# espiriki/Garbage_Classification_RCA

Hardware: AMD Instinct MI355X
Metric: train samples/sec (image+text pairs), MM-RCA ViT-B16+DistilBERT (higher is better)
Workload: dtype bf16

## Files before the change

garbage_classification_rca_amd/csrc/gemm256.hip:

```cpp
#include "common.h"
#include "lds_asm.h"
#include <type_traits>
#include <mutex>

typedef __attribute__((ext_vector_type(4))) float f32x4;
typedef __attribute__((address_space(3))) void lds_void;
typedef const __attribute__((address_space(1))) void gbl_void;

#define HT_BYTES (128 * 64 * 2)
#define STAGE_BYTES (4 * HT_BYTES)
#define LDS256_BYTES (128 * (256 * 4 + 16))
#define SLOT_A0 0
#define SLOT_A1 1
#define SLOT_B0 2
#define SLOT_B1 3

__device__ __forceinline__ int krow_f2(int row) { return (row & 3) | (((row >> 3) & 1) << 2); }

__device__ __forceinline__ void stage_half(const bf16_t* src0, const bf16_t* src1, char* lds_piece0) {
  __builtin_amdgcn_global_load_lds((gbl_void*)src0, (lds_void*)(lds_piece0), 16, 0, 0);
  __builtin_amdgcn_global_load_lds((gbl_void*)src1, (lds_void*)(lds_piece0 + 1024), 16, 0, 0);
}

template <bool F4>
__device__ __forceinline__ void stage_half_t(const bf16_t* src0, const bf16_t* src1, char* lds_piece0) {
  __builtin_amdgcn_global_load_lds((gbl_void*)src0, (lds_void*)(lds_piece0), 16, 0, 0);
  __builtin_amdgcn_global_load_lds((gbl_void*)src1, (lds_void*)(lds_piece0 + (F4 ? 8192 : 1024)), 16, 0, 0);
}

template <bool KROW, bool STRIPE = false>
__device__ __forceinline__ const bf16_t* piece_src(const bf16_t* __restrict__ base, int64_t ld, int64_t row0, int64_t rows_total,
                                                   int i, int lane, int h = 0) {
  if (!KROW) {
    const int r = 8 * i + (lane >> 3);
    const int c = (lane & 7) ^ ((r >> 1) & 7);
    int64_t gr = row0 + (STRIPE ? 64 * (r >> 5) + 32 * h + (r & 31) : r);
// ... 818 lines not shown
                       lda, ldb, ldc, tiles_m, tiles_n, ksteps_base, ksteps_rem, (float*)workspace, (float*)nullptr, splits,    \
                       (const bf16_t*)A_lo, (const bf16_t*)B_lo, nseg);                                                         \
  } while (0)
  if (x3) {
    if (!ak && !bk) LSLAB(false, false, true);
    else if (!ak && bk) LSLAB(false, true, true);
    else if (ak && !bk) LSLAB(true, false, true);
    else LSLAB(true, true, true);
  } else {
    if (!ak && !bk) LSLAB(false, false, false);
    else if (!ak && bk) LSLAB(false, true, false);
    else if (ak && !bk) LSLAB(true, false, false);
    else LSLAB(true, true, false);
  }
#undef LSLAB
  MMRCA_CHECK_LAUNCH("gemm_splitk(mfma256)");
  hipLaunchKernelGGL(splitk_reduce256_k, dim3(tiles * 64), dim3(256), 0, st, (const float*)workspace, C, ldc, tiles, tiles_n, splits, M, N);
  MMRCA_CHECK_LAUNCH("gemm_splitk(reduce)");
  return 0;
}

extern "C" int mmrca_gemm_splitk(const void* A, const void* B, float* C, void* workspace, int64_t workspace_bytes, int64_t M,
                                 int64_t N, int64_t K, int64_t lda, int64_t ldb, int64_t ldc, int a_layout, int b_layout,
                                 void* stream) {
  return gemm_splitk_impl(A, nullptr, B, nullptr, C, workspace, workspace_bytes, M, N, K, lda, ldb, ldc, a_layout, b_layout, stream);
}

extern "C" int mmrca_gemm_splitk_x3(const void* A_hi, const void* A_lo, const void* B_hi, const void* B_lo, float* C, void* workspace,
                                    int64_t workspace_bytes, int64_t M, int64_t N, int64_t K, int64_t lda, int64_t ldb, int64_t ldc,
                                    int a_layout, int b_layout, void* stream) {
  MMRCA_REQUIRE(A_lo || !B_lo, "gemm_x3(splitk): a B lo plane without an A lo plane is not a supported pass set");
  return gemm_splitk_impl(A_hi, A_lo, B_hi, B_lo, C, workspace, workspace_bytes, M, N, K, lda, ldb, ldc, a_layout, b_layout, stream);
}
```

garbage_classification_rca_amd/engine.py:

```python
from __future__ import annotations

import math
import os
import re
from typing import Dict, List, Optional, Tuple

import torch

from . import lib as L
from . import spec as S
from .conv_engine import ConvEncoder, CONV_MODELS

ALIGN = 64
CONCURRENT_ENCODERS = os.environ.get("MMRCA_CONCURRENT_ENCODERS", "1") == "1"
CLS_TAIL = os.environ.get("MMRCA_CLS_TAIL", "1") == "1"
X3_WGRAD_PASSES = int(os.environ.get("MMRCA_X3_WGRAD_PASSES", "3"))
X3_DGRAD_PASSES = int(os.environ.get("MMRCA_X3_DGRAD_PASSES", "3"))
ROWPAD = 256


def _round_up(x: int, m: int) -> int:
    return (x + m - 1) // m * m


class Arena:
    def __init__(self, entries: List[Tuple[str, Tuple[int, ...]]], device, with_lp: bool, with_lo: bool = False):
        self.offsets: Dict[str, Tuple[int, Tuple[int, ...], int]] = {}
        off = 0
        for k, shp in entries:
            n = 1
            for s in shp:
                n *= s
            off = _round_up(off, ALIGN)
            self.offsets[k] = (off, tuple(shp), n)
            off += n
        self.total = _round_up(off, ALIGN)
        self.p = torch.zeros(self.total, dtype=torch.float32, device=device)
        self.g = torch.zeros(self.total, dtype=torch.float32, device=device)
        self.lp = torch.zeros(self.total, dtype=torch.bfloat16, device=device) if with_lp else None
        self.lp_lo = torch.zeros(self.total, dtype=torch.bfloat16, device=device) if with_lo else None
        self.lp_valid = False
        self._views: Dict[Tuple[str, str], torch.Tensor] = {}

    def view(self, key, which="p"):
        v = self._views.get((key, which))
        if v is None:
            off, shp, n = self.offsets[key]
            v = self._views[(key, which)] = getattr(self, which)[off:off + n].view(shp)
# ... 285 lines not shown
                elif is_norm:
                    v.fill_(1.0 if leaf == "weight" else 0.0)
                elif is_head:
                    if v.dim() == 2:
                        bound = 1.0 / math.sqrt(v.shape[1])
                        v.copy_((torch.rand(v.shape, generator=g) * 2 - 1) * bound)
                        self._last_fan_in = v.shape[1]
                    else:
                        bound = 1.0 / math.sqrt(self._last_fan_in)
                        v.copy_((torch.rand(v.shape, generator=g) * 2 - 1) * bound)
                elif leaf == "bias" or leaf.endswith("_bias"):
                    v.zero_()
                else:
                    v.copy_(torch.randn(v.shape, generator=g) * 0.02)
        self.arena.lp_valid = False

    def load_arrays(self, sd: Dict[str, "torch.Tensor"], strict=True):
        with torch.no_grad():
            for k in self.param_keys:
                if k in sd:
                    self.arena.view(k).copy_(torch.as_tensor(sd[k]).to(self.device, torch.float32).view(self.arena.offsets[k][1]))
                elif strict:
                    raise KeyError(k)
        self.arena.lp_valid = False

    def _splitk_ws(self):
        key = ("splitk_ws", torch.cuda.current_stream().cuda_stream)
        t = self._bufs.get(key)
        if t is None:
            t = torch.empty(L.SPLITK_WS_BYTES, dtype=torch.uint8, device=self.device)
            self._bufs[key] = t
        return t

    def vec(self, name, n, dtype=torch.float32, layer=0):
        key = (name, layer, "vec", n, dtype)
        t = self._bufs.get(key)
        if t is None:
            t = self._bufs[key] = torch.zeros(1, n, dtype=dtype, device=self.device)
        return t

    def buf(self, name, rows, cols, dtype=None, layer=0):
        dtype = dtype or self.dtype
        key = (name, layer, rows, cols, dtype)
        t = self._bufs.get(key)
        if t is None:
            t = torch.zeros(_round_up(max(rows, 1), ROWPAD), cols, dtype=dtype, device=self.device)
            self._bufs[key] = t
        return t

    def release_buffers(self):
        self.buffer_generation += 1
        self._bufs.clear()
        self._plane_valid.clear()
        self._plane_fresh.clear()
        self._saved = None
        if self.conv is not None:
            self.conv.release()

    def _lin_fwd(self, x, wkey, bkey, out, M, N, K, act=L.ACT_NONE, preact=None, addend=None, wnumel=None):
        if self.x3:
            b = self.arena.view(bkey) if wnumel is None else self.arena.p[self.arena.offsets[bkey][0]:self.arena.offsets[bkey][0] + N]
            po = isinstance(out, Planes)
            L.gemm_x3(self._split(x, M, K), self.Wx3(wkey, wnumel), out.hi if po else out, C_lo=(out.lo if po else None), bias=b, addend=addend,
                      preact=preact, M=M, N=N, K=K, lda=K, ldb=K, ldc=N, a_layout=L.ROWK, b_layout=L.ROWK, act=act, impl=self.gemm_impl)
            return
        w = self.W(wkey) if wnumel is None else self.Wflat(wkey, wnumel)
        b = self.W(bkey) if wnumel is None else self.Wflat(bkey, N)
        L.gemm(x, w, out, bias=b, addend=addend, preact=preact, M=M, N=N, K=K, lda=K, ldb=K, ldc=N,
               a_layout=L.ROWK, b_layout=L.ROWK, act=act, dtype=self.dt, impl=self.gemm_impl)

    def _lin_bwd(self, dy, x, wkey, bkey, dx, M, N, K, addend=None, wnumel=None, gelu_h=None, bias_done=False, gelu_db=None):
        Mk = _round_up(M, 64)
        gw = self.G(wkey) if wnumel is None else self.Gflat(wkey, wnumel)
        gb = self.G(bkey) if wnumel is None else self.Gflat(bkey, N)
        if self.x3 and not self.x3f:
            return self._lin_bwd_x3(dy, x, wkey, dx, M, N, K, Mk, gw, gb, addend, wnumel, gelu_h, bias_done, gelu_db)
        if self.x3f:
            x = self._hi(x, M, K)
        bdt = self.bdt
        if self.gemm_impl == L.IMPL_AUTO and L.gemm_splitk_ok(N, K, Mk, bdt):
            L.gemm_splitk(dy, x, gw, self._splitk_ws(), M=N, N=K, K=Mk, lda=N, ldb=K, ldc=K)
        else:
            L.gemm(dy, x, gw, M=N, N=K, K=Mk, lda=N, ldb=K, ldc=K, a_layout=L.KROW, b_layout=L.KROW, accum=True, dtype=bdt,
                   impl=self.gemm_impl)
        if not bias_done:
            L.colsum_accum(dy, gb, M, N, N, bdt)
        if dx is not None:
            w = self.Wb(wkey, wnumel)
            fuse = gelu_h is not None
            L.gemm(dy, w, dx, addend=addend, preact=(gelu_h if fuse else None), M=M, N=K, K=N, lda=N, ldb=K, ldc=K,
                   a_layout=L.ROWK, b_layout=L.KROW, act=(L.ACT_MUL if fuse else L.ACT_NONE), dtype=bdt,
                   impl=self.gemm_impl, colsum=(gelu_db if fuse else None))

    def _lin_bwd_x3(self, dy, x, wkey, dx, M, N, K, Mk, gw, gb, addend, wnumel, gelu_h, bias_done, gelu_db):
        dyp = self._split(dy, M, N)
        xp = self._split(x, M, K, reuse=True)
        wg_a, wg_b = (dyp, xp) if X3_WGRAD_PASSES >= 3 else ((dyp, (xp[0], None)) if X3_WGRAD_PASSES == 2 else ((dyp[0], None), (xp[0], None)))
        if self.gemm_impl == L.IMPL_AUTO and L.gemm_splitk_ok(N, K, Mk, L.BF16):
            L.gemm_splitk_x3(wg_a, wg_b, gw, self._splitk_ws(), M=N, N=K, K=Mk, lda=N, ldb=K, ldc=K)
        else:
            L.gemm_x3(wg_a, wg_b, gw, M=N, N=K, K=Mk, lda=N, ldb=K, ldc=K, a_layout=L.KROW, b_layout=L.KROW, accum=True)
        if not bias_done:
            if isinstance(dy, Planes):
                raise L.MmrcaError("bf16x3: the bias gradient of a two-plane dY must come from its producer (bias_done)")
            L.colsum_accum(dy, gb, M, N, N, self.dt)
        if dx is not None:
            fuse = gelu_h is not None
            po = isinstance(dx, Planes)
            wp = self.Wx3(wkey, wnumel)
            dg_a, dg_b = (dyp, wp) if X3_DGRAD_PASSES >= 3 else ((dyp, (wp[0], None)) if X3_DGRAD_PASSES == 2 else ((dyp[0], None), (wp[0], None)))
            L.gemm_x3(dg_a, dg_b, dx.hi if po else dx, C_lo=(dx.lo if po else None), addend=addend,
                      preact=(gelu_h if fuse else None), colsum=(gelu_db if fuse else None),
                      M=M, N=K, K=N, lda=N, ldb=K, ldc=K, a_layout=L.ROWK, b_layout=L.KROW, act=(L.ACT_MUL if fuse else L.ACT_NONE),
                      impl=self.gemm_impl)

    def _ln_fwd(self, x, res, pfx, sum_out, y, mean, rstd, rows, D, eps, ld_x=None, ld_y=None, in_drop=(0.0, 0), out_drop=(0.0, 0),
                to_gemm=False):
# ... 109 lines not shown
                h, g = cb("h", Fd, self._hdt), (self.planes_buf("t_g_c", B, Fd, i if save else 0) if self._g_planes else cb("g", Fd))
                self._lin_fwd(x1, P + K["f1"] + ".weight", P + K["f1"] + ".bias", g, B, Fd, D, act=self._gelu_act, preact=h)
                f = cb("f", D)
                self._lin_fwd(g, P + K["f2"] + ".weight", P + K["f2"] + ".bias", f, B, D, Fd)
                s2, xn = cb("s2", D), cb("xout", D)
                m2, r2 = stat("m2c", i), stat("r2c", i)
                self._ln_fwd(f, x1, P + K["ln2"], s2, xn, m2, r2, B, D, s.ln_eps, in_drop=(dp, sd(i, 3)))
                layers.append(dict(x=x, qkv=qkv, ctx=ctx, lse=lse, s1=s1, x1=x1, m1=m1, r1=r1, h=h, g=g, s2=s2, m2=m2, r2=r2,
                                   ctx_c=ctx_c, tail=True))
                cls = xn[:B].clone()
                return cls, dict(B=B, T=T, M=M, cu=cu, first=first, ids32=ids32, pos=pos, mask32=mask32, emb=emb, mean0=mean0, rstd0=rstd0, layers=layers,
                                 drop_p=dp, drop_seed=drop_seed, taps=tap_rows)
            self._mha_fwd(qkv, mask32, ctx, lse, B, H, T, dh, drop_p=dp, drop_seed=sd(i, 1), cu=cu)
            att = fb("tmpD", D)
            self._lin_fwd(ctx, P + K["o"] + ".weight", P + K["o"] + ".bias", att, M, D, D)
            s1, x1 = fb("s1", D, i), fb("x1", D, i)
            m1, r1 = stat("m1", i), stat("r1", i)
            self._ln_fwd(att, x, P + K["ln1"], s1, x1, m1, r1, M, D, s.ln_eps, in_drop=(post_attn_drop, sd(i, 2)), to_gemm=True)
            h, g = fb("h", Fd, i, self._hdt), (self.planes_buf("t_g", cap, Fd, i if save else 0) if self._g_planes else fb("g", Fd, i))
            self._lin_fwd(x1, P + K["f1"] + ".weight", P + K["f1"] + ".bias", g, M, Fd, D, act=self._gelu_act, preact=h)
            f = fb("tmpD", D)
            self._lin_fwd(g, P + K["f2"] + ".weight", P + K["f2"] + ".bias", f, M, D, Fd)
            s2, xn = fb("s2", D, i), fb("x", D, i + 1)
            m2, r2 = stat("m2", i), stat("r2", i)
            self._ln_fwd(f, x1, P + K["ln2"], s2, xn, m2, r2, M, D, s.ln_eps, in_drop=(dp, sd(i, 3)), to_gemm=(i + 1 < s.layers))
            layers.append(dict(x=x, qkv=qkv, ctx=ctx, lse=lse, s1=s1, x1=x1, m1=m1, r1=r1, h=h, g=g, s2=s2, m2=m2, r2=r2))
            x = xn
            if taps and (i + 1) in taps:
                tap_rows[i + 1] = x.index_select(0, first)
        cls = x.index_select(0, first)
        return cls, dict(B=B, T=T, M=M, cu=cu, first=first, ids32=ids32, pos=pos, mask32=mask32, emb=emb, mean0=mean0, rstd0=rstd0, layers=layers,
                         drop_p=dp, drop_seed=drop_seed, taps=tap_rows)

    def _text_upper_backward(self, dy, sv, i, K, rows, cap, sfx):
        s, P = self.ts, "text_model."
        D, Fd = s.dim, s.ffn
        a = sv["layers"][i]
        gb = lambda name, cols: self.buf("tg_" + name + sfx, cap, cols, self.gdtype)
        dp, sd = sv["drop_p"], (lambda layer, site: self._site_seed(sv["drop_seed"], layer, site))
        post_attn_drop = dp if s.name != "distilbert" else 0.0
        ds2 = gb("ds2", D)
        df = gb("dbr_ffn", D) if dp > 0 else None
        gb_f2, gb_o = self.G(P + K["f2"] + ".bias"), self.G(P + K["o"] + ".bias")
        self._ln_bwd(dy, a["s2"], P + K["ln2"], a["m2"], a["r2"], None, ds2, rows, D, branch_drop=(dp, sd(i, 3)), dbranch=df,
                     dcol=(None if df is not None else gb_f2), dcol_branch=(gb_f2 if df is not None else None))
        dg = self.planes_buf("tg_dF" + sfx, cap, Fd) if (self._g_planes and not self.x3f) else gb("dF", Fd)
        self._lin_bwd(df if df is not None else ds2, a["g"], P + K["f2"] + ".weight", P + K["f2"] + ".bias", dg, rows, D, Fd,
                      gelu_h=a["h"], bias_done=True, gelu_db=self.G(P + K["f1"] + ".bias"))
        dx1 = gb("dxB", D)
        self._lin_bwd(dg, a["x1"], P + K["f1"] + ".weight", P + K["f1"] + ".bias", dx1, rows, Fd, D, addend=ds2, bias_done=True)
        ds1 = gb("ds1", D)
        datt = gb("dbr_att", D) if post_attn_drop > 0 else None
        self._ln_bwd(dx1, a["s1"], P + K["ln1"], a["m1"], a["r1"], None, ds1, rows, D, branch_drop=(post_attn_drop, sd(i, 2)), dbranch=datt,
                     dcol=(None if datt is not None else gb_o), dcol_branch=(gb_o if datt is not None else None))
        dctx = gb("dctx", D)
        self._lin_bwd(datt if datt is not None else ds1, a["ctx_c" if sfx else "ctx"], P + K["o"] + ".weight", P + K["o"] + ".bias", dctx,
                      rows, D, D, bias_done=True)
        return ds1, dctx

    def _text_backward(self, dcls, sv, dtaps=None):
        s, P = self.ts, "text_model."
        B, T = sv["B"], sv["T"]
        M, D, H = sv["M"], s.dim, s.heads
        dh, cu, first = D // H, sv["cu"], sv["first"]
        gb = lambda name, cols: self.buf("tg_" + name, B * T, cols, self.gdtype)
        dx = gb("dxA", D)
        tail = bool(sv["layers"][-1].get("tail"))
        if not tail:
            dx[:M].zero_()
            dx.index_copy_(0, first, dcls.to(dx.dtype))
        for i in reversed(range(s.layers)):
            if tail and i == s.layers - 1:
                self._text_backward_tail(dcls, sv, dx)
                continue
            K, a = S.text_layer_keys(s, i), sv["layers"][i]
            if dtaps and (i + 1) in dtaps:
                dx.index_add_(0, first, dtaps[i + 1].to(dx.dtype))
            ds1, dctx = self._text_upper_backward(dx, sv, i, K, M, B * T, "")
            dqkv = gb("dqkv", 3 * D)
            qkv_b, ctx_b = self._attn_bwd_operands(a, M, D, "tg", B * T, B)
            L.mha_bwd(qkv_b, sv["mask32"], ctx_b, dctx, a["lse"], dqkv, B, H, T, dh, dh ** -0.5, self.bdt, self.attn_impl,
                      drop_p=sv["drop_p"], drop_seed=self._site_seed(sv["drop_seed"], i, 1), cu=cu)
            self._lin_bwd(dqkv, a["x"], P + K["q"] + ".weight", P + K["q"] + ".bias", dx, M, 3 * D, D, addend=ds1, wnumel=3 * D * D)
            self._ready(f"text_layer_{i}")
        ds0 = gb("ds2", D)
        self._ln_bwd(dx, sv["emb"], P + "embeddings.LayerNorm", sv["mean0"], sv["rstd0"], None, ds0, M, D,
                     dy_drop=(sv["drop_p"], self._site_seed(sv["drop_seed"], 0, 0)))
        dtype_row = self.Gflat(P + "embeddings.token_type_embeddings.weight", D) if s.type_vocab else None
        L.embed_bwd(ds0, sv["ids32"], sv["pos"], self.G(P + "embeddings.word_embeddings.weight"),
                    self.G(P + "embeddings.position_embeddings.weight"), dtype_row, M, D, self.bdt,
                    pad_id=s.pad_id, pos_pad_id=(s.pad_id if s.pos_offset else -1))
        self._ready("text_emb", flush=True)

    def _text_backward_tail(self, dcls, sv, dx):
        s, P = self.ts, "text_model."
        B, T = sv["B"], sv["T"]
        M, D, H = sv["M"], s.dim, s.heads
        dh, i, cu, first = D // H, s.layers - 1, sv["cu"], sv["first"]
        K, a = S.text_layer_keys(s, i), sv["layers"][i]
        gb = lambda name, cols: self.buf("tg_" + name, B * T, cols, self.gdtype)
        dxc = self.buf("tg_dx_c", B, D, self.gdtype)
        dxc[:B].copy_(dcls)
        ds1, dctx_c = self._text_upper_backward(dxc, sv, i, K, B, B, "_c")
        ds1_full = gb("ds1", D)
        ds1_full[:M].zero_()
        ds1_full.index_copy_(0, first, ds1[:B])
        dqkv = gb("dqkv", 3 * D)
        qkv_b, ctx_b = self._attn_bwd_operands(a, M, D, "tg", B * T, B)
        L.mha_cls_bwd(qkv_b, sv["mask32"], ctx_b, dctx_c, a["lse"], dqkv, B, H, T, dh, dh ** -0.5, self.bdt,
                      drop_p=sv["drop_p"], drop_seed=self._site_seed(sv["drop_seed"], i, 1), cu=cu)
        self._lin_bwd(dqkv, a["x"], P + K["q"] + ".weight", P + K["q"] + ".bias", dx, M, 3 * D, D, addend=ds1_full, wnumel=3 * D * D)
        self._ready(f"text_layer_{i}")

    def _vision_forward(self, images, save):
        s, P = self.vs, "image_model."
        B = images.shape[0]
# ... 47 lines not shown
                mf, rf = stat("mf"), stat("rf")
                self._ln_fwd(xn, None, P + "encoder.ln", None, feat, mf, rf, B, D, s.ln_eps)
                return feat[:B], dict(B=B, patches=patches, xL=xn, mf=mf, rf=rf, layers=layers)
            self._mha_fwd(qkv, None, ctx, lse, B, H, Tn, dh)
            x1 = fb("x1", M, D, i)
            y2, m2, r2 = (self.planes_buf("v_y2", M, D, i if save else 0) if self._ln_planes else fb("y2", M, D, i)), stat("m2", i), stat("r2", i)
            if fuse_res:
                ao = fb("attn_o", M, D, 0)
                self._lin_fwd(ctx, Lk + "self_attention.out_proj.weight", Lk + "self_attention.out_proj.bias", ao, M, D, D)
                self._ln_fwd(ao, x, Lk + "ln_2", x1, y2, m2, r2, M, D, s.ln_eps)
            else:
                self._lin_fwd(ctx, Lk + "self_attention.out_proj.weight", Lk + "self_attention.out_proj.bias", x1, M, D, D, addend=x)
                self._ln_fwd(x1, None, Lk + "ln_2", None, y2, m2, r2, M, D, s.ln_eps)
            h, g = fb("h", M, Fd, i, self._hdt), (self.planes_buf("v_g", M, Fd, i if save else 0) if self._g_planes else fb("g", M, Fd, i))
            self._lin_fwd(y2, Lk + "mlp.0.weight", Lk + "mlp.0.bias", g, M, Fd, D, act=self._gelu_act, preact=h)
            layers.append(dict(x=x, y1=y1, m1=m1, r1=r1, qkv=qkv, ctx=ctx, lse=lse, x1=x1, y2=y2, m2=m2, r2=r2, h=h, g=g))
            if fuse_res:
                f2 = fb("ffn_o", M, D, 0)
                self._lin_fwd(g, Lk + "mlp.3.weight", Lk + "mlp.3.bias", f2, M, D, Fd)
                pend = (f2, x1)
            else:
                xn = fb("x", M, D, i + 1)
                self._lin_fwd(g, Lk + "mlp.3.weight", Lk + "mlp.3.bias", xn, M, D, Fd, addend=x1)
                x = xn
        feat = self.buf("v_feat", B, D)
        mf, rf = stat("mf"), stat("rf")
        if pend is None:
            self._ln_fwd(x, None, P + "encoder.ln", None, feat, mf, rf, B, D, s.ln_eps, ld_x=Tn * D, ld_y=D)
        else:
            x = fb("x", M, D, s.layers)
            self._ln_fwd(pend[0], pend[1], P + "encoder.ln", x, feat, mf, rf, B, D, s.ln_eps, ld_x=Tn * D, ld_y=D)
        return feat[:B], dict(B=B, patches=patches, xL=x, mf=mf, rf=rf, layers=layers)

    def _vision_upper_backward(self, dx, sv, i, rows, sfx):
        s = self.vs
        D, Fd = s.dim, s.ffn
        Lk, a = f"image_model.encoder.layers.encoder_layer_{i}.", sv["layers"][i]
        gb = lambda name, cols: self.buf("vg_" + name + sfx, rows, cols, self.gdtype)
        dg = self.planes_buf("vg_dF" + sfx, rows, Fd) if (self._g_planes and not self.x3f) else gb("dF", Fd)
        self._lin_bwd(dx, a["g"], Lk + "mlp.3.weight", Lk + "mlp.3.bias", dg, rows, D, Fd, gelu_h=a["h"], bias_done=True,
                      gelu_db=self.G(Lk + "mlp.0.bias"))
        dy2 = gb("dy", D)
        self._lin_bwd(dg, a["y2"], Lk + "mlp.0.weight", Lk + "mlp.0.bias", dy2, rows, Fd, D, bias_done=True)
        dx1 = gb("dxB", D)
        self._ln_bwd(dy2, a["x1"], Lk + "ln_2", a["m2"], a["r2"], dx, dx1, rows, D, dcol=self.G(Lk + "self_attention.out_proj.bias"))
        dctx = gb("dctx", D)
        self._lin_bwd(dx1, a["ctx_c" if sfx else "ctx"], Lk + "self_attention.out_proj.weight", Lk + "self_attention.out_proj.bias", dctx,
                      rows, D, D, bias_done=True)
        return dctx, dx1

    def _vision_backward(self, dfeat, sv):
        s, P = self.vs, "image_model."
        B = sv["B"]
        nP, Tn, D, H = s.tokens - 1, s.tokens, s.dim, s.heads
        dh, M, Kp = D // H, B * Tn, 3 * s.patch * s.patch
        gb = lambda name, rows, cols: self.buf("vg_" + name, rows, cols, self.gdtype)
        dx = gb("dxA", M, D)
        dfe = gb("dfeat", B, D)
        dfe[:B].copy_(dfeat)
        top = P + f"encoder.layers.encoder_layer_{s.layers - 1}."
        tail = bool(sv["layers"][-1].get("tail"))
        if tail:
            dxc = gb("dx_c", B, D)
            self._ln_bwd(dfe, sv["xL"], P + "encoder.ln", sv["mf"], sv["rf"], None, dxc, B, D, dcol=self.G(top + "mlp.3.bias"))
        else:
            dx[:M].zero_()
            self._ln_bwd(dfe, sv["xL"], P + "encoder.ln", sv["mf"], sv["rf"], None, dx, B, D, ld_dy=D, ld_s=Tn * D, ld_ds=Tn * D,
                         dcol=self.G(top + "mlp.3.bias"))
        self._ready("image_ln")
        for i in reversed(range(s.layers)):
            if tail and i == s.layers - 1:
                self._vision_backward_tail(dxc, sv, dx)
                continue
            Lk, a = P + f"encoder.layers.encoder_layer_{i}.", sv["layers"][i]
            dctx, dx1 = self._vision_upper_backward(dx, sv, i, M, "")
            dqkv = gb("dqkv", M, 3 * D)
            qkv_b, ctx_b = self._attn_bwd_operands(a, M, D, "vg", M, B)
            L.mha_bwd(qkv_b, None, ctx_b, dctx, a["lse"], dqkv, B, H, Tn, dh, dh ** -0.5, self.bdt, self.attn_impl)
            dy1 = gb("dy", M, D)
            self._lin_bwd(dqkv, a["y1"], Lk + "self_attention.in_proj_weight", Lk + "self_attention.in_proj_bias", dy1, M, 3 * D, D)
            below = P + f"encoder.layers.encoder_layer_{i - 1}.mlp.3.bias"
            self._ln_bwd(dy1, a["x"], Lk + "ln_1", a["m1"], a["r1"], dx1, dx, M, D, dcol=(self.G(below) if i > 0 else None))
            self._ready(f"image_layer_{i}")
        dproj = gb("dproj", B * nP, D)
        L.vit_assemble_bwd(dx, dproj, self.Gflat(P + "class_token", D), self.Gflat(P + "encoder.pos_embedding", Tn * D), B, nP, D, self.bdt)
        self._lin_bwd(dproj, sv["patches"], P + "conv_proj.weight", P + "conv_proj.bias", None, B * nP, D, Kp, wnumel=D * Kp)
        self._ready("image_emb", flush=True)

    def _vision_backward_tail(self, dxc, sv, dx):
        s, P = self.vs, "image_model."
        B = sv["B"]
        Tn, D, H = s.tokens, s.dim, s.heads
        dh, M, i = D // H, B * Tn, s.layers - 1
        Lk, a = P + f"encoder.layers.encoder_layer_{i}.", sv["layers"][i]
        gb = lambda name, rows, cols: self.buf("vg_" + name, rows, cols, self.gdtype)
        dctx_c, dx1c = self._vision_upper_backward(dxc, sv, i, B, "_c")
        dx1 = gb("dxB", M, D)
        dx1[:M].zero_()
        dx1[:M].view(B, Tn, D)[:, 0] = dx1c[:B]
        dqkv = gb("dqkv", M, 3 * D)
        qkv_b, ctx_b = self._attn_bwd_operands(a, M, D, "vg", M, B)
        L.mha_cls_bwd(qkv_b, None, ctx_b, dctx_c, a["lse"], dqkv, B, H, Tn, dh, dh ** -0.5, self.bdt)
        dy1 = gb("dy", M, D)
        self._lin_bwd(dqkv, a["y1"], Lk + "self_attention.in_proj_weight", Lk + "self_attention.in_proj_bias", dy1, M, 3 * D, D)
        below = P + f"encoder.layers.encoder_layer_{i - 1}.mlp.3.bias"
        self._ln_bwd(dy1, a["x"], Lk + "ln_1", a["m1"], a["r1"], dx1, dx, M, D, dcol=(self.G(below) if i > 0 else None))
        self._ready(f"image_layer_{i}")

    def _check_resident(self, *named):
        for t, nm in named:
            if t is None or not t.is_cuda:
                raise L.MmrcaError(f"{nm} must be in HBM; the {self.PATH_NAME} path has no CPU fallback")

# ... 104 lines not shown
```

Baseline: 6892.

## Group same-K weight-gradient GEMMs into one stream-K split-K launch

Adds a grouped stream-K split-K weight-gradient GEMM kernel that processes up to four products sharing the reduction dimension in a single launch. Work units are balanced across workgroups, with partial tiles written to a slab and summed by one reduce kernel. The engine defers wgrad GEMMs for the FFN pair and for the out_proj+qkv pair in the ViT and text backward passes, then flushes them as one group. This targets launch overhead and poor CU fill from small per-layer split-K GEMMs, at the cost of a larger workspace and an extra pass over the partial slab.

Result: no change. 6883 (-0.1%).

```diff
diff --git a/garbage_classification_rca_amd/csrc/gemm256.hip b/garbage_classification_rca_amd/csrc/gemm256.hip
--- a/garbage_classification_rca_amd/csrc/gemm256.hip
+++ b/garbage_classification_rca_amd/csrc/gemm256.hip
@@ -1,7 +1,10 @@
 #include "common.h"
 #include "lds_asm.h"
+#include "../../include/mmrca_wgrad.h"
 #include <type_traits>
 #include <mutex>
+#include <algorithm>
+#include <string.h>
 
 typedef __attribute__((ext_vector_type(4))) float f32x4;
 typedef __attribute__((address_space(3))) void lds_void;
@@ -886,3 +889,233 @@
   MMRCA_REQUIRE(A_lo || !B_lo, "gemm_x3(splitk): a B lo plane without an A lo plane is not a supported pass set");
   return gemm_splitk_impl(A_hi, A_lo, B_hi, B_lo, C, workspace, workspace_bytes, M, N, K, lda, ldb, ldc, a_layout, b_layout, stream);
 }
+
+#define SKG_MAX_PROBLEMS 4
+#define SKG_MAX_WG 256
+#define SKG_MAX_TILES 1024
+struct SkgProblem {
+  const bf16_t* A;
+  const bf16_t* B;
+  float* C;
+  int64_t M, N, lda, ldb, ldc;
+  int tiles_m, tiles_n, tile0;
+  int colmajor;
+};
+struct SkgArgs {
+  SkgProblem p[SKG_MAX_PROBLEMS];
+  int count, T, S, W;
+  int g, P;
+  unsigned short order[SKG_MAX_WG];
+};
+
+__host__ __device__ __forceinline__ int64_t skg_boundary(int w, int W, int S, int64_t U) {
+  if (w <= 0) return 0;
+  if (w >= W) return U;
+  int64_t x = (int64_t)w * U / W;
+  const int r = (int)(x % S);
+  if (r == 1) x -= 1;
+  else if (r == S - 1) x += 1;
+  return x;
+}
+__host__ __device__ __forceinline__ int skg_tile_at(int i, int g, int P) { return (i % P) * g + i / P; }
+__host__ __device__ __forceinline__ int skg_position_of(int t, int g, int P) { return (t % g) * P + t / g; }
+__host__ __device__ __forceinline__ int skg_range_of(int64_t u, int W, int S, int64_t U) {
+  int w = (int)(u * W / U);
+  if (w > W - 1) w = W - 1;
+  while (w > 0 && skg_boundary(w, W, S, U) > u) --w;
+  while (w < W - 1 && skg_boundary(w + 1, W, S, U) <= u) ++w;
+  return w;
+}
+static inline int skg_workgroups(int max_workgroups, int64_t U) {
+  int64_t W = max_workgroups > 0 ? max_workgroups : cu_count();
+  if (W > SKG_MAX_WG) W = SKG_MAX_WG;
+  if (W > U / 3) W = U / 3;
+  return W < 1 ? 1 : (int)W;
+}
+
+template <bool X3 = false>
+__global__ void __launch_bounds__(512, 2)
+gemm_splitk_group256_k(const SkgArgs g, float* __restrict__ slab) {
+  constexpr bool A_KROW = true, B_KROW = true;
+  extern __shared__ __attribute__((aligned(16))) char smem[];
+  const int wave = __builtin_amdgcn_readfirstlane(threadIdx.x >> 6), lane = threadIdx.x & 63;
+  const int wr = wave >> 2, wc = wave & 3;
+
+  const int per_xcd = (g.W + 7) >> 3;
+  const int rank = ((int)blockIdx.x & 7) * per_xcd + ((int)blockIdx.x >> 3);
+  if (((int)blockIdx.x >> 3) >= per_xcd || rank >= g.W) return;
+  const int w = g.order[rank];
+  const int S = g.S;
+  const int64_t U = (int64_t)g.T * S;
+  int64_t u = skg_boundary(w, g.W, S, U);
+  const int64_t u_end = skg_boundary(w + 1, g.W, S, U);
+
+  f32x4 acc[2][2][4][2];
+  int64_t a_step = 0, b_step = 0;
+  const bf16_t* pa[2][2];
+  const bf16_t* pb[2][2];
+  char* const my_piece = smem + wave * 2048;
+  int issue_stage = 0;
+  [[maybe_unused]] int issue_kt = 0, issue_seg = 0;
+  [[maybe_unused]] const int ksteps_seg = 0, nseg = 0;
+  [[maybe_unused]] auto repoint = [](int, int64_t) {};
+
+  const unsigned lds0 = (unsigned)(uintptr_t)(lds_void*)smem;
+  const int gq = lane >> 4, l16 = lane & 15;
+  unsigned abase[4], bbase[2];
+  {
+    const int q = l16 >> 2, p = l16 & 3, row = 8 * gq + q;
+#pragma unroll
+    for (int i = 0; i < 4; ++i) abase[i] = lds0 + row * 256 + ((((4 * wr + i) ^ krow_f2(row))) << 5) + p * 8;
+#pragma unroll
+    for (int j = 0; j < 2; ++j) bbase[j] = lds0 + row * 256 + ((((2 * wc + j) ^ krow_f2(row))) << 5) + p * 8;
+  }
+  Frag<A_KROW> af[4][2];
+  Frag<B_KROW> b0f[2][2], b1f[2][2];
+  [[maybe_unused]] unsigned read_stage = 0;
+
+  while (u < u_end) {
+    const int pos = (int)(u / S);
+    const int t = skg_tile_at(pos, g.g, g.P);
+    const int k0 = (int)(u - (int64_t)pos * S);
+    const int64_t tile_end = (int64_t)(pos + 1) * S;
+    const int64_t seg_end = u_end < tile_end ? u_end : tile_end;
+    const int nt = (int)(seg_end - u);
+    const bf16_t* A = g.p[0].A; const bf16_t* B = g.p[0].B;
+    int64_t M = g.p[0].M, N = g.p[0].N, lda = g.p[0].lda, ldb = g.p[0].ldb;
+    int tiles_m = g.p[0].tiles_m, tiles_n = g.p[0].tiles_n, tile0 = 0, colmajor = g.p[0].colmajor;
+#pragma unroll
+    for (int q = 1; q < SKG_MAX_PROBLEMS; ++q)
+      if (q < g.count && t >= g.p[q].tile0) {
+        A = g.p[q].A; B = g.p[q].B; M = g.p[q].M; N = g.p[q].N; lda = g.p[q].lda; ldb = g.p[q].ldb;
+        tiles_m = g.p[q].tiles_m; tiles_n = g.p[q].tiles_n; tile0 = g.p[q].tile0; colmajor = g.p[q].colmajor;
+      }
+    const int tl = t - tile0;
+    const int tm = colmajor ? tl % tiles_m : tl / tiles_n, tn = colmajor ? tl / tiles_m : tl % tiles_n;
+    const int64_t m_blk = (int64_t)tm * 256, n_blk = (int64_t)tn * 256;
+    a_step = 64 * lda; b_step = 64 * ldb;
+#pragma unroll
+    for (int h = 0; h < 2; ++h)
+#pragma unroll
+      for (int ii = 0; ii < 2; ++ii) {
+        pa[h][ii] = piece_src<true>(A, lda, m_blk + 128 * h, M, wave * 2 + ii, lane) + (int64_t)k0 * 64 * lda;
+        pb[h][ii] = piece_src<true>(B, ldb, n_blk + 128 * h, N, wave * 2 + ii, lane) + (int64_t)k0 * 64 * ldb;
+      }
+#pragma unroll
+    for (int a = 0; a < 2; ++a)
+#pragma unroll
+      for (int b = 0; b < 2; ++b)
+#pragma unroll
+        for (int i = 0; i < 4; ++i)
+#pragma unroll
+          for (int j = 0; j < 2; ++j) acc[a][b][i][j] = (f32x4){0.f, 0.f, 0.f, 0.f};
+
+    ISSUE(0); ISSUE(1); ISSUE(2); ISSUE(3); ISSUE(0); ISSUE(1);
+    VMCNT(8);
+    BARRIER();
+    if (wr) BARRIER();
+    __builtin_amdgcn_sched_barrier(0);
+
+    for (int kt = 0; kt < nt - 2; ++kt) K_TILE_G(ISSUE, 1, 1, 1, 1, 8, 8, 10, 8);
+    K_TILE_G(ISSUE, 1, 1, 0, 0, 8, 8, 8, 4);
+    K_TILE_G(ISSUE, 0, 0, 0, 0, 2, 0, 0, 0);
+    if (!wr) BARRIER();
+
+    float* dst = slab + (int64_t)(w + pos) * 65536 + wave * 8192 + lane * 4;
+#pragma unroll
+    for (int a = 0; a < 2; ++a)
+#pragma unroll
+      for (int b = 0; b < 2; ++b)
+#pragma unroll
+        for (int i = 0; i < 4; ++i)
+#pragma unroll
+          for (int j = 0; j < 2; ++j)
+            *reinterpret_cast<f32x4*>(dst + (((a * 2 + b) * 4 + i) * 2 + j) * 256) = acc[a][b][i][j];
+    VMCNT(0);
+    u = seg_end;
+  }
+}
+
+__global__ void __launch_bounds__(256)
+splitk_group_reduce256_k(const SkgArgs g, const float* __restrict__ slab) {
+  const int tile = blockIdx.x >> 6;
+  const int idx = ((blockIdx.x & 63) << 8) + threadIdx.x;
+  const int S = g.S;
+  const int64_t U = (int64_t)g.T * S;
+  const int pos = skg_position_of(tile, g.g, g.P);
+  const int w0 = skg_range_of((int64_t)pos * S, g.W, S, U), w1 = skg_range_of((int64_t)(pos + 1) * S - 1, g.W, S, U);
+  const float* src = slab + (int64_t)pos * 65536 + (int64_t)idx * 4;
+  f32x4 s = *reinterpret_cast<const f32x4*>(src + (int64_t)w0 * 65536);
+  for (int w = w0 + 1; w <= w1; ++w) {
+    const f32x4 v = *reinterpret_cast<const f32x4*>(src + (int64_t)w * 65536);
+    s += v;
+  }
+  float* C = g.p[0].C;
+  int64_t ldc = g.p[0].ldc;
+  int tiles_m = g.p[0].tiles_m, tiles_n = g.p[0].tiles_n, tile0 = 0, colmajor = g.p[0].colmajor;
+#pragma unroll
+  for (int q = 1; q < SKG_MAX_PROBLEMS; ++q)
+    if (q < g.count && tile >= g.p[q].tile0) {
+      C = g.p[q].C; ldc = g.p[q].ldc; tiles_m = g.p[q].tiles_m; tiles_n = g.p[q].tiles_n; tile0 = g.p[q].tile0; colmajor = g.p[q].colmajor;
+    }
+  const int wv = idx >> 11, f = (idx >> 6) & 31, lane = idx & 63;
+  const int a = f >> 4, b = (f >> 3) & 1, i = (f >> 1) & 3, j = f & 1;
+  const int wr = wv >> 2, wc = wv & 3, l16 = lane & 15, gq = lane >> 4;
+  const int row = 128 * a + 64 * wr + 16 * i + l16, col = 128 * b + 32 * wc + 16 * j + 4 * gq;
+  const int tl = tile - tile0;
+  const int tm = colmajor ? tl % tiles_m : tl / tiles_n, tn = colmajor ? tl / tiles_m : tl % tiles_n;
+  float* dst = C + ((int64_t)tm * 256 + row) * ldc + (int64_t)tn * 256 + col;
+  f32x4 c = *reinterpret_cast<f32x4*>(dst);
+  c += s;
+  *reinterpret_cast<f32x4*>(dst) = c;
+}
+
+extern "C" int64_t mmrca_gemm_splitk_group_workspace_bytes(int64_t tiles, int max_workgroups) {
+  if (tiles <= 0 || tiles > SKG_MAX_TILES || max_workgroups < 0) return 0;
+  int64_t W = max_workgroups > 0 ? max_workgroups : cu_count();
+  if (W > SKG_MAX_WG) W = SKG_MAX_WG;
+  return (W + tiles) * 65536 * 4;
+}
+
+extern "C" int mmrca_gemm_splitk_group(const MmrcaWgradProblem* problems, int count, int64_t K, void* workspace, int64_t workspace_bytes,
+                                       int max_workgroups, void* stream) {
+  MMRCA_REQUIRE(problems && count >= 1 && count <= SKG_MAX_PROBLEMS, "gemm_splitk_group: needs 1 to %d products (got %d)", SKG_MAX_PROBLEMS, count);
+  MMRCA_REQUIRE(K >= 128 && K % 64 == 0 && K / 64 < (1 << 24), "gemm_splitk_group: needs K %% 64 == 0 and K >= 128 (got K=%lld)", (long long)K);
+  MMRCA_REQUIRE(workspace && max_workgroups >= 0, "gemm_splitk_group: null workspace or negative max_workgroups");
+  SkgArgs g;
+  memset(&g, 0, sizeof(g));
+  int64_t tiles = 0;
+  for (int q = 0; q < count; ++q) {
+    const MmrcaWgradProblem& p = problems[q];
+    MMRCA_REQUIRE(p.A && p.B && p.C, "gemm_splitk_group: null operand in product %d", q);
+    MMRCA_REQUIRE(p.M > 0 && p.N > 0 && p.M % 256 == 0 && p.N % 256 == 0,
+                  "gemm_splitk_group: M and N must be multiples of 256 (product %d: M=%lld N=%lld)", q, (long long)p.M, (long long)p.N);
+    MMRCA_REQUIRE(p.lda % 8 == 0 && p.ldb % 8 == 0 && p.ldc % 4 == 0 &&
+                  (((uintptr_t)p.A | (uintptr_t)p.B | (uintptr_t)p.C | (uintptr_t)workspace) & 15) == 0,
+                  "gemm_splitk_group: operands must be 16-byte aligned (product %d)", q);
+    MMRCA_REQUIRE(p.lda >= p.M && p.ldb >= p.N && p.ldc >= p.N, "gemm_splitk_group: leading dimension too small (product %d)", q);
+    MMRCA_REQUIRE(tiles + (p.M / 256) * (p.N / 256) <= SKG_MAX_TILES, "gemm_splitk_group: more than %d output tiles", SKG_MAX_TILES);
+    g.p[q] = SkgProblem{(const bf16_t*)p.A, (const bf16_t*)p.B, p.C, p.M, p.N, p.lda, p.ldb, p.ldc, (int)(p.M / 256), (int)(p.N / 256),
+                        (int)tiles, p.M > p.N ? 1 : 0};
+    tiles += (p.M / 256) * (p.N / 256);
+  }
+  const int S = (int)(K / 64), T = (int)tiles;
+  const int64_t U = (int64_t)T * S;
+  const int W = skg_workgroups(max_workgroups, U);
+  g.count = count; g.T = T; g.S = S; g.W = W;
+  g.g = T;
+  for (int b = W; b != 0;) { const int r = g.g % b; g.g = b; b = r; }
+  g.P = T / g.g;
+  const int64_t need = (int64_t)(W + T - 1) * 65536 * 4;
+  MMRCA_REQUIRE(workspace_bytes >= need, "gemm_splitk_group: workspace too small (%lld < %lld bytes)", (long long)workspace_bytes, (long long)need);
+  int key[SKG_MAX_WG];
+  for (int w = 0; w < W; ++w) { key[w] = (int)(skg_boundary(w, W, S, U) % S); g.order[w] = (unsigned short)w; }
+  std::stable_sort(g.order, g.order + W, [&](unsigned short a, unsigned short b) { return key[a] < key[b]; });
+  hipStream_t st = (hipStream_t)stream;
+  MMRCA_MAX_LDS(LDS256_BYTES, gemm_splitk_group256_k<false>);
+  hipLaunchKernelGGL((gemm_splitk_group256_k<false>), dim3((W + 7) / 8 * 8), dim3(512), LDS256_BYTES, st, g, (float*)workspace);
+  MMRCA_CHECK_LAUNCH("gemm_splitk_group(mfma256)");
+  hipLaunchKernelGGL(splitk_group_reduce256_k, dim3(T * 64), dim3(256), 0, st, g, (const float*)workspace);
+  MMRCA_CHECK_LAUNCH("gemm_splitk_group(reduce)");
+  return 0;
+}
diff --git a/garbage_classification_rca_amd/engine.py b/garbage_classification_rca_amd/engine.py
--- a/garbage_classification_rca_amd/engine.py
+++ b/garbage_classification_rca_amd/engine.py
@@ -9,11 +9,14 @@
 
 from . import lib as L
 from . import spec as S
+from . import wgrad as WG
 from .conv_engine import ConvEncoder, CONV_MODELS
 
 ALIGN = 64
 CONCURRENT_ENCODERS = os.environ.get("MMRCA_CONCURRENT_ENCODERS", "1") == "1"
 CLS_TAIL = os.environ.get("MMRCA_CLS_TAIL", "1") == "1"
+WGRAD_GROUP = os.environ.get("MMRCA_WGRAD_GROUP", "1") != "0"
+WGRAD_GROUP_MAX_BYTES = 512 << 20
 X3_WGRAD_PASSES = int(os.environ.get("MMRCA_X3_WGRAD_PASSES", "3"))
 X3_DGRAD_PASSES = int(os.environ.get("MMRCA_X3_DGRAD_PASSES", "3"))
 ROWPAD = 256
@@ -365,6 +368,27 @@
             self._bufs[key] = t
         return t
 
+    def _splitk_group_ws(self, tiles):
+        key = ("splitk_group_ws", torch.cuda.current_stream().cuda_stream)
+        need = WG.workspace_bytes(tiles)
+        t = self._bufs.get(key)
+        if t is None or t.numel() < need:
+            t = torch.empty(need, dtype=torch.uint8, device=self.device)
+            self._bufs[key] = t
+        return t
+
+    def _wgrad_pair_ok(self, cols, rows):
+        return WGRAD_GROUP and 2 * cols * _round_up(rows, 64) <= WGRAD_GROUP_MAX_BYTES
+
+    def _wgrad_flush(self, pend):
+        if len(pend) > 1 and len({p[5] for p in pend}) == 1 and len(pend) <= WG.MAX_PRODUCTS:
+            tiles = sum((N // 256) * (K // 256) for _, _, _, N, K, _ in pend)
+            WG.gemm_splitk_group([(dy, x, gw, N, K, N, K, K) for dy, x, gw, N, K, _ in pend], self._splitk_group_ws(tiles), K=pend[0][5])
+        else:
+            for dy, x, gw, N, K, Mk in pend:
+                L.gemm_splitk(dy, x, gw, self._splitk_ws(), M=N, N=K, K=Mk, lda=N, ldb=K, ldc=K)
+        pend.clear()
+
     def vec(self, name, n, dtype=torch.float32, layer=0):
         key = (name, layer, "vec", n, dtype)
         t = self._bufs.get(key)
@@ -402,7 +426,8 @@
         L.gemm(x, w, out, bias=b, addend=addend, preact=preact, M=M, N=N, K=K, lda=K, ldb=K, ldc=N,
                a_layout=L.ROWK, b_layout=L.ROWK, act=act, dtype=self.dt, impl=self.gemm_impl)
 
-    def _lin_bwd(self, dy, x, wkey, bkey, dx, M, N, K, addend=None, wnumel=None, gelu_h=None, bias_done=False, gelu_db=None):
+    def _lin_bwd(self, dy, x, wkey, bkey, dx, M, N, K, addend=None, wnumel=None, gelu_h=None, bias_done=False, gelu_db=None,
+                 wg=None, wg_flush=True):
         Mk = _round_up(M, 64)
         gw = self.G(wkey) if wnumel is None else self.Gflat(wkey, wnumel)
         gb = self.G(bkey) if wnumel is None else self.Gflat(bkey, N)
@@ -412,10 +437,15 @@
             x = self._hi(x, M, K)
         bdt = self.bdt
         if self.gemm_impl == L.IMPL_AUTO and L.gemm_splitk_ok(N, K, Mk, bdt):
-            L.gemm_splitk(dy, x, gw, self._splitk_ws(), M=N, N=K, K=Mk, lda=N, ldb=K, ldc=K)
+            if wg is not None:
+                wg.append((dy, x, gw, N, K, Mk))
+            else:
+                L.gemm_splitk(dy, x, gw, self._splitk_ws(), M=N, N=K, K=Mk, lda=N, ldb=K, ldc=K)
         else:
             L.gemm(dy, x, gw, M=N, N=K, K=Mk, lda=N, ldb=K, ldc=K, a_layout=L.KROW, b_layout=L.KROW, accum=True, dtype=bdt,
                    impl=self.gemm_impl)
+        if wg and wg_flush:
+            self._wgrad_flush(wg)
         if not bias_done:
             L.colsum_accum(dy, gb, M, N, N, bdt)
         if dx is not None:
@@ -591,9 +621,10 @@
         return cls, dict(B=B, T=T, M=M, cu=cu, first=first, ids32=ids32, pos=pos, mask32=mask32, emb=emb, mean0=mean0, rstd0=rstd0, layers=layers,
                          drop_p=dp, drop_seed=drop_seed, taps=tap_rows)
 
-    def _text_upper_backward(self, dy, sv, i, K, rows, cap, sfx):
+    def _text_upper_backward(self, dy, sv, i, K, rows, cap, sfx, wg=None):
         s, P = self.ts, "text_model."
         D, Fd = s.dim, s.ffn
+        ffn = [] if (not sfx and self._wgrad_pair_ok(2 * (D + Fd), rows)) else None
         a = sv["layers"][i]
         gb = lambda name, cols: self.buf("tg_" + name + sfx, cap, cols, self.gdtype)
         dp, sd = sv["drop_p"], (lambda layer, site: self._site_seed(sv["drop_seed"], layer, site))
@@ -605,16 +636,16 @@
                      dcol=(None if df is not None else gb_f2), dcol_branch=(gb_f2 if df is not None else None))
         dg = self.planes_buf("tg_dF" + sfx, cap, Fd) if (self._g_planes and not self.x3f) else gb("dF", Fd)
         self._lin_bwd(df if df is not None else ds2, a["g"], P + K["f2"] + ".weight", P + K["f2"] + ".bias", dg, rows, D, Fd,
-                      gelu_h=a["h"], bias_done=True, gelu_db=self.G(P + K["f1"] + ".bias"))
+                      gelu_h=a["h"], bias_done=True, gelu_db=self.G(P + K["f1"] + ".bias"), wg=ffn, wg_flush=False)
         dx1 = gb("dxB", D)
-        self._lin_bwd(dg, a["x1"], P + K["f1"] + ".weight", P + K["f1"] + ".bias", dx1, rows, Fd, D, addend=ds2, bias_done=True)
+        self._lin_bwd(dg, a["x1"], P + K["f1"] + ".weight", P + K["f1"] + ".bias", dx1, rows, Fd, D, addend=ds2, bias_done=True, wg=ffn)
         ds1 = gb("ds1", D)
         datt = gb("dbr_att", D) if post_attn_drop > 0 else None
         self._ln_bwd(dx1, a["s1"], P + K["ln1"], a["m1"], a["r1"], None, ds1, rows, D, branch_drop=(post_attn_drop, sd(i, 2)), dbranch=datt,
                      dcol=(None if datt is not None else gb_o), dcol_branch=(gb_o if datt is not None else None))
         dctx = gb("dctx", D)
         self._lin_bwd(datt if datt is not None else ds1, a["ctx_c" if sfx else "ctx"], P + K["o"] + ".weight", P + K["o"] + ".bias", dctx,
-                      rows, D, D, bias_done=True)
+                      rows, D, D, bias_done=True, wg=wg, wg_flush=False)
         return ds1, dctx
 
     def _text_backward(self, dcls, sv, dtaps=None):
@@ -635,12 +666,13 @@
             K, a = S.text_layer_keys(s, i), sv["layers"][i]
             if dtaps and (i + 1) in dtaps:
                 dx.index_add_(0, first, dtaps[i + 1].to(dx.dtype))
-            ds1, dctx = self._text_upper_backward(dx, sv, i, K, M, B * T, "")
+            wg = [] if self._wgrad_pair_ok(6 * D, M) else None
+            ds1, dctx = self._text_upper_backward(dx, sv, i, K, M, B * T, "", wg=wg)
             dqkv = gb("dqkv", 3 * D)
             qkv_b, ctx_b = self._attn_bwd_operands(a, M, D, "tg", B * T, B)
             L.mha_bwd(qkv_b, sv["mask32"], ctx_b, dctx, a["lse"], dqkv, B, H, T, dh, dh ** -0.5, self.bdt, self.attn_impl,
                       drop_p=sv["drop_p"], drop_seed=self._site_seed(sv["drop_seed"], i, 1), cu=cu)
-            self._lin_bwd(dqkv, a["x"], P + K["q"] + ".weight", P + K["q"] + ".bias", dx, M, 3 * D, D, addend=ds1, wnumel=3 * D * D)
+            self._lin_bwd(dqkv, a["x"], P + K["q"] + ".weight", P + K["q"] + ".bias", dx, M, 3 * D, D, addend=ds1, wnumel=3 * D * D, wg=wg)
             self._ready(f"text_layer_{i}")
         ds0 = gb("ds2", D)
         self._ln_bwd(dx, sv["emb"], P + "embeddings.LayerNorm", sv["mean0"], sv["rstd0"], None, ds0, M, D,
@@ -754,21 +786,22 @@
             self._ln_fwd(pend[0], pend[1], P + "encoder.ln", x, feat, mf, rf, B, D, s.ln_eps, ld_x=Tn * D, ld_y=D)
         return feat[:B], dict(B=B, patches=patches, xL=x, mf=mf, rf=rf, layers=layers)
 
-    def _vision_upper_backward(self, dx, sv, i, rows, sfx):
+    def _vision_upper_backward(self, dx, sv, i, rows, sfx, wg=None):
         s = self.vs
         D, Fd = s.dim, s.ffn
+        ffn = [] if (not sfx and self._wgrad_pair_ok(2 * (D + Fd), rows)) else None
         Lk, a = f"image_model.encoder.layers.encoder_layer_{i}.", sv["layers"][i]
         gb = lambda name, cols: self.buf("vg_" + name + sfx, rows, cols, self.gdtype)
         dg = self.planes_buf("vg_dF" + sfx, rows, Fd) if (self._g_planes and not self.x3f) else gb("dF", Fd)
         self._lin_bwd(dx, a["g"], Lk + "mlp.3.weight", Lk + "mlp.3.bias", dg, rows, D, Fd, gelu_h=a["h"], bias_done=True,
-                      gelu_db=self.G(Lk + "mlp.0.bias"))
+                      gelu_db=self.G(Lk + "mlp.0.bias"), wg=ffn, wg_flush=False)
         dy2 = gb("dy", D)
-        self._lin_bwd(dg, a["y2"], Lk + "mlp.0.weight", Lk + "mlp.0.bias", dy2, rows, Fd, D, bias_done=True)
+        self._lin_bwd(dg, a["y2"], Lk + "mlp.0.weight", Lk + "mlp.0.bias", dy2, rows, Fd, D, bias_done=True, wg=ffn)
         dx1 = gb("dxB", D)
         self._ln_bwd(dy2, a["x1"], Lk + "ln_2", a["m2"], a["r2"], dx, dx1, rows, D, dcol=self.G(Lk + "self_attention.out_proj.bias"))
         dctx = gb("dctx", D)
         self._lin_bwd(dx1, a["ctx_c" if sfx else "ctx"], Lk + "self_attention.out_proj.weight", Lk + "self_attention.out_proj.bias", dctx,
-                      rows, D, D, bias_done=True)
+                      rows, D, D, bias_done=True, wg=wg, wg_flush=False)
         return dctx, dx1
 
     def _vision_backward(self, dfeat, sv):
@@ -795,12 +828,13 @@
                 self._vision_backward_tail(dxc, sv, dx)
                 continue
             Lk, a = P + f"encoder.layers.encoder_layer_{i}.", sv["layers"][i]
-            dctx, dx1 = self._vision_upper_backward(dx, sv, i, M, "")
+            wg = [] if self._wgrad_pair_ok(6 * D, M) else None
+            dctx, dx1 = self._vision_upper_backward(dx, sv, i, M, "", wg=wg)
             dqkv = gb("dqkv", M, 3 * D)
             qkv_b, ctx_b = self._attn_bwd_operands(a, M, D, "vg", M, B)
             L.mha_bwd(qkv_b, None, ctx_b, dctx, a["lse"], dqkv, B, H, Tn, dh, dh ** -0.5, self.bdt, self.attn_impl)
             dy1 = gb("dy", M, D)
-            self._lin_bwd(dqkv, a["y1"], Lk + "self_attention.in_proj_weight", Lk + "self_attention.in_proj_bias", dy1, M, 3 * D, D)
+            self._lin_bwd(dqkv, a["y1"], Lk + "self_attention.in_proj_weight", Lk + "self_attention.in_proj_bias", dy1, M, 3 * D, D, wg=wg)
             below = P + f"encoder.layers.encoder_layer_{i - 1}.mlp.3.bias"
             self._ln_bwd(dy1, a["x"], Lk + "ln_1", a["m1"], a["r1"], dx1, dx, M, D, dcol=(self.G(below) if i > 0 else None))
             self._ready(f"image_layer_{i}")
diff --git a/garbage_classification_rca_amd/wgrad.py b/garbage_classification_rca_amd/wgrad.py
--- /dev/null
+++ b/garbage_classification_rca_amd/wgrad.py
@@ -0,0 +1,114 @@
+from __future__ import annotations
+
+import ctypes as C
+import math
+import os
+from typing import List, NamedTuple, Sequence, Tuple
+
+from . import abi
+from . import lib as L
+
+HEADER_PATH = os.path.join(os.path.dirname(os.path.dirname(os.path.abspath(__file__))), "include", "mmrca_wgrad.h")
+FUNCTIONS = ("mmrca_gemm_splitk_group", "mmrca_gemm_splitk_group_workspace_bytes")
+MAX_PRODUCTS, MAX_WORKGROUPS, MAX_TILES, TILE_BYTES = 4, 256, 1024, 256 * 256 * 4
+SNAP_ALLOWANCE = 2
+
+
+class WgradProblem(C.Structure):
+    _fields_ = [("A", C.c_void_p), ("B", C.c_void_p), ("C", C.c_void_p), ("M", C.c_int64), ("N", C.c_int64),
+                ("lda", C.c_int64), ("ldb", C.c_int64), ("ldc", C.c_int64)]
+
+
+_typed = None
+
+
+def _fns():
+    global _typed
+    lib = L.load()
+    if _typed is not lib:
+        protos = abi.prototypes(HEADER_PATH, {"MmrcaWgradProblem": C.POINTER(WgradProblem)})
+        if tuple(sorted(protos)) != tuple(sorted(FUNCTIONS)):
+            raise L.MmrcaError(f"{HEADER_PATH} declares {sorted(protos)}, this module binds {sorted(FUNCTIONS)}")
+        for name, (restype, params) in protos.items():
+            fn = getattr(lib, name)
+            fn.restype, fn.argtypes = restype, [ctype for ctype, _ in params]
+        _typed = lib
+    return lib
+
+
+class Plan(NamedTuple):
+    W: int
+    T: int
+    S: int
+    bounds: List[int]
+    segments: List[Tuple[int, int, int, int, int]]
+
+
+def workgroups(tiles: int, ksteps: int, max_workgroups: int) -> int:
+    return max(1, min(max_workgroups, MAX_WORKGROUPS, tiles * ksteps // 3))
+
+
+def boundary(w: int, W: int, S: int, U: int) -> int:
+    if w <= 0:
+        return 0
+    if w >= W:
+        return U
+    x = w * U // W
+    r = x % S
+    if r == 1:
+        x -= 1
+    elif r == S - 1:
+        x += 1
+    return x
+
+
+def tile_at(i: int, T: int, W: int) -> int:
+    g = math.gcd(T, W)
+    P = T // g
+    return (i % P) * g + i // P
+
+
+def position_of(t: int, T: int, W: int) -> int:
+    g = math.gcd(T, W)
+    return (t % g) * (T // g) + t // g
+
+
+def plan(tiles: int, K: int, max_workgroups: int) -> Plan:
+    if tiles < 1 or K < 128 or K % 64 or max_workgroups < 1:
+        raise ValueError(f"plan: needs tiles >= 1, K % 64 == 0, K >= 128 and max_workgroups >= 1 (got {tiles}, {K}, {max_workgroups})")
+    S = K // 64
+    U = tiles * S
+    W = workgroups(tiles, S, max_workgroups)
+    bounds = [boundary(w, W, S, U) for w in range(W + 1)]
+    segments = []
+    for w in range(W):
+        u = bounds[w]
+        while u < bounds[w + 1]:
+            pos = u // S
+            end = min(bounds[w + 1], (pos + 1) * S)
+            segments.append((w, tile_at(pos, tiles, W), u - pos * S, end - u, w + pos))
+            u = end
+    return Plan(W, tiles, S, bounds, segments)
+
+
+def workspace_bytes(tiles: int, max_workgroups: int = 0) -> int:
+    return int(_fns().mmrca_gemm_splitk_group_workspace_bytes(tiles, max_workgroups))
+
+
+def gemm_splitk_group(products: Sequence[tuple], workspace, *, K: int, max_workgroups: int = 0):
+    n = len(products)
+    arr = (WgradProblem * max(n, 1))()
+    for q, (A, B, Cout, M, N, lda, ldb, ldc) in enumerate(products):
+        L._dev(A, "gemm_splitk_group A")
+        if A.shape[0] < K or B.shape[0] < K:
+            raise L.MmrcaError(f"gemm_splitk_group: product {q} has operands of {A.shape[0]} and {B.shape[0]} rows, the group's K is {K}")
+        arr[q] = WgradProblem(L.ptr(A), L.ptr(B), L.ptr(Cout), M, N, lda, ldb, ldc)
+    prof = L.GEMM_PROFILE is not None
+    if prof:
+        e0, e1 = L._events()
+    L._check(_fns().mmrca_gemm_splitk_group(arr, n, K, L.ptr(workspace), workspace.numel() * workspace.element_size(),
+                                            max_workgroups, L.stream_ptr()), "mmrca_gemm_splitk_group")
+    if prof:
+        e1.record()
+        mn = sum(p[3] * p[4] for p in products)
+        L.GEMM_PROFILE.append((2.0 * mn * K, (L.KROW, L.KROW, 1), e0, e1, (mn // 256, 256, K, L.ACT_NONE)))
diff --git a/include/mmrca_wgrad.h b/include/mmrca_wgrad.h
--- /dev/null
+++ b/include/mmrca_wgrad.h
@@ -0,0 +1,24 @@
+#ifndef MMRCA_WGRAD_H
+#define MMRCA_WGRAD_H
+#include <stdint.h>
+#ifdef __cplusplus
+extern "C" {
+#endif
+
+typedef struct {
+  const void* A;
+  const void* B;
+  float* C;
+  int64_t M, N;
+  int64_t lda, ldb, ldc;
+} MmrcaWgradProblem;
+
+int64_t mmrca_gemm_splitk_group_workspace_bytes(int64_t tiles, int max_workgroups);
+
+int mmrca_gemm_splitk_group(const MmrcaWgradProblem* problems, int count, int64_t K, void* workspace, int64_t workspace_bytes,
+                            int max_workgroups, void* stream);
+
+#ifdef __cplusplus
+}
+#endif
+#endif
```
